# shaneson0/attacking_federate_learning

Measured on AMD Instinct MI355X. Metric: aggregation rounds/sec at N clients x D params (Bulyan), higher is better.
Workload: dtype f32 (Gram: fp16x2 split of every fp32 operand, 3 fp16 MFMAs per block, fp32/fp64 accumulate; <= 2e-7 of |gi||gj| vs f...

## Files before the change

### attacking_federate_learning_amd/csrc/gram_planes.hip

```cpp
#include "common.hpp"

#include <cstring>
#include <type_traits>

namespace byz {
namespace {

constexpr int kWgRows = 256;
constexpr int kWgCols = 128;
constexpr int kSlab = 128;
constexpr int kThreads = 512;
constexpr int kFragBytes = 1024;
constexpr int kRowBlocks = (kWgRows + kWgCols) / 32;
constexpr int kChunkCols = 8192;
constexpr int kChunkSteps = kChunkCols / 16;
constexpr int kFlushSteps = 16;
constexpr int kSpareRoundsPercent = 10;

typedef float f32x16 __attribute__((ext_vector_type(16)));
typedef float f32x4 __attribute__((ext_vector_type(4)));
typedef __bf16 bf16x8 __attribute__((ext_vector_type(8)));
typedef _Float16 f16x8 __attribute__((ext_vector_type(8)));
typedef uint32_t u32x4 __attribute__((ext_vector_type(4)));

__device__ __forceinline__ void split_bf16x3(const f32x4& lo4, const f32x4& hi4, u32x4& hp, u32x4& mp, u32x4& lp) {
    uint32_t xb[8], r1b[8], r2b[8];
#pragma unroll
    for (int e = 0; e < 8; ++e) {
        const float x = e < 4 ? lo4[e] : hi4[e - 4];
        xb[e] = __float_as_uint(x);
        const float r1 = x - __uint_as_float(xb[e] & 0xffff0000u);
        r1b[e] = __float_as_uint(r1);
        const float r2 = r1 - __uint_as_float(r1b[e] & 0xffff0000u);
        r2b[e] = __float_as_uint(r2);
    }
#pragma unroll
    for (int e = 0; e < 4; ++e) {
        hp[e] = __builtin_amdgcn_perm(xb[2 * e + 1], xb[2 * e], 0x07060302u);
        mp[e] = __builtin_amdgcn_perm(r1b[2 * e + 1], r1b[2 * e], 0x07060302u);
        lp[e] = __builtin_amdgcn_perm(r2b[2 * e + 1], r2b[2 * e], 0x07060302u);
    }
}

__device__ __forceinline__ void split_f16x2(const f32x4& lo4, const f32x4& hi4, float scale, u32x4& hp, u32x4& mp) {
    f16x8 h, m;
#pragma unroll
    for (int e = 0; e < 8; ++e) {
        const float x = (e < 4 ? lo4[e] : hi4[e - 4]) * scale;
        h[e] = static_cast<_Float16>(x);
        m[e] = static_cast<_Float16>(x - static_cast<float>(h[e]));
    }
    hp = __builtin_bit_cast(u32x4, h);
    mp = __builtin_bit_cast(u32x4, m);
}

__device__ __forceinline__ f32x4 load4_tail(const float* __restrict__ src, int64_t k, int64_t n_cols) {
    f32x4 v = {0.0f, 0.0f, 0.0f, 0.0f};
    if (k + 3 < n_cols) {
        v = *reinterpret_cast<const f32x4*>(src + k);
    } else {
        if (k + 0 < n_cols) v.x = src[k + 0];
        if (k + 1 < n_cols) v.y = src[k + 1];
        if (k + 2 < n_cols) v.z = src[k + 2];
    }
    return v;
}

constexpr int kSplitCols = 128;
__global__ __launch_bounds__(256) void plane_split_bf16_kernel(const float* __restrict__ G, int64_t n_rows, int64_t n_cols,
                                                               int64_t ld, const int32_t* __restrict__ row_index,
                                                               int64_t k0, int64_t n_steps, u32x4* __restrict__ planes) {
    __shared__ __attribute__((aligned(16))) float tile[32][kSplitCols + 4];
    const int tid = threadIdx.x;
    const int64_t rb = blockIdx.y;
    const int64_t step0 = static_cast<int64_t>(blockIdx.x) * (kSplitCols / 16);
    {
        const int r = tid >> 3, c = tid & 7;
        int64_t row = rb * 32 + r;
        if (row > n_rows - 1) row = n_rows - 1;
        if (row_index != nullptr) row = row_index[row];
        const float* src = G + row * ld;
#pragma unroll
        for (int p = 0; p < 4; ++p) {
            const int col = 4 * c + 32 * p;
            *reinterpret_cast<f32x4*>(&tile[r][col]) = load4_tail(src, k0 + step0 * 16 + col, n_cols);
        }
    }
    __syncthreads();
    const int lane = tid & 63, wave = tid >> 6;
#pragma unroll
    for (int i = 0; i < 2; ++i) {
        const int sl = 2 * wave + i;
        const int64_t step = step0 + sl;
        if (step >= n_steps) continue;
        const int row = lane & 31, kk = sl * 16 + 8 * (lane >> 5);
        const f32x4 lo4 = *reinterpret_cast<const f32x4*>(&tile[row][kk]);
        const f32x4 hi4 = *reinterpret_cast<const f32x4*>(&tile[row][kk + 4]);
        u32x4 h, m, l;
        split_bf16x3(lo4, hi4, h, m, l);
        u32x4* out = planes + ((rb * n_steps + step) * 3) * 64 + lane;
        out[0] = h;
        out[64] = m;
        out[128] = l;
    }
}

__global__ __launch_bounds__(256) void plane_split_f16_kernel(const float* __restrict__ G, int64_t n_rows, int64_t n_cols,
                                                              int64_t ld, const int32_t* __restrict__ row_index, int64_t k0,
                                                              int64_t n_steps, u32x4* __restrict__ planes,
                                                              double* __restrict__ unscale, int64_t rows_pad,
                                                              const int32_t* __restrict__ redo) {
    __shared__ __attribute__((aligned(16))) float tile[32][kSplitCols + 4];
    __shared__ float row_scale[32];
    const int tid = threadIdx.x;
    const int lane = tid & 63, wave = tid >> 6;
    const int listed = redo != nullptr ? redo[0] : 1;
    for (int item = redo != nullptr ? static_cast<int>(blockIdx.x) : 0; item < listed; item += static_cast<int>(gridDim.x)) {
    const int64_t rb = redo != nullptr ? redo[2 + 2 * item] : blockIdx.y;
    const int64_t chunk = redo != nullptr ? redo[1 + 2 * item] : blockIdx.x;
    const int r = tid >> 3, c = tid & 7;
    int64_t row = rb * 32 + r;
    if (row > n_rows - 1) row = n_rows - 1;
    if (row_index != nullptr) row = row_index[row];
    const float* src = G + row * ld;
    const int64_t kbeg = k0 + chunk * kChunkCols;
    {
        float mx = 0.0f;
        bool bad = false;
#pragma unroll 8
        for (int i = 0; i < kChunkCols / 32; ++i) {
            const f32x4 v = load4_tail(src, kbeg + 4 * c + 32 * i, n_cols);
#pragma unroll
            for (int e = 0; e < 4; ++e) {
                const float a = __builtin_fabsf(v[e]);
                bad = bad || !(a <= 3.0e38f);
                mx = __builtin_fmaxf(mx, a);
            }
        }
#pragma unroll
        for (int msk = 1; msk < 8; msk <<= 1) {
            mx = __builtin_fmaxf(mx, __shfl_xor(mx, msk, 64));
            bad = bad || (__shfl_xor(bad ? 1 : 0, msk, 64) != 0);
        }
        int shift = 0;
        if (!bad && mx > 0.0f) {
            shift = 14 - (static_cast<int>((__float_as_uint(mx) >> 23) & 0xffu) - 127);
            if (mx < 1.17549435e-38f) shift = 126;
            if (shift > 126) shift = 126;
            if (shift < -126) shift = -126;
        }
        if (c == 0) {
            row_scale[r] = __uint_as_float(static_cast<uint32_t>(shift + 127) << 23);
            unscale[chunk * rows_pad + rb * 32 + r] = __longlong_as_double(static_cast<long long>(1023 - shift) << 52);
        }
    }
    __syncthreads();
    const int64_t step_base = chunk * kChunkSteps;
    for (int sub = 0; sub < kChunkCols / kSplitCols; ++sub) {
        const int64_t step0 = step_base + sub * (kSplitCols / 16);
        if (step0 >= n_steps) break;
#pragma unroll
        for (int p = 0; p < 4; ++p) {
            const int col = 4 * c + 32 * p;
            *reinterpret_cast<f32x4*>(&tile[r][col]) = load4_tail(src, k0 + step0 * 16 + col, n_cols);
        }
        __syncthreads();
#pragma unroll
        for (int i = 0; i < 2; ++i) {
            const int sl = 2 * wave + i;
            const int64_t step = step0 + sl;
            if (step >= n_steps) continue;
            const int frow = lane & 31, kk = sl * 16 + 8 * (lane >> 5);
            const f32x4 lo4 = *reinterpret_cast<const f32x4*>(&tile[frow][kk]);
            const f32x4 hi4 = *reinterpret_cast<const f32x4*>(&tile[frow][kk + 4]);
            u32x4 h, m;
            split_f16x2(lo4, hi4, row_scale[frow], h, m);
            u32x4* out = planes + ((rb * n_steps + step) * 2) * 64 + lane;
            out[0] = h;
            out[64] = m;
        }
        __syncthreads();
    }
    if (redo == nullptr) break;
    __syncthreads();
    }
}

constexpr int kSampleGroups = 16;
__global__ __launch_bounds__(256) void plane_split_f16_stream_kernel(const float* __restrict__ G, int64_t n_rows, int64_t n_cols,
                                                                     int64_t ld, const int32_t* __restrict__ row_index, int64_t k0,
                                                                     int64_t n_steps, u32x4* __restrict__ planes,
                                                                     double* __restrict__ unscale, int64_t rows_pad,
                                                                     int32_t* __restrict__ redo) {
    __shared__ __attribute__((aligned(16))) float tile[2][32][kSplitCols + 4];
    __shared__ float row_scale[32];
    __shared__ int block_bad;
    const int tid = threadIdx.x;
    const int lane = tid & 63, wave = tid >> 6;
    const int64_t rb = blockIdx.y;
    const int64_t chunk = blockIdx.x;
    const int r = tid >> 3, c = tid & 7;
    int64_t row = rb * 32 + r;
    if (row > n_rows - 1) row = n_rows - 1;
    if (row_index != nullptr) row = row_index[row];
    const float* src = G + row * ld;
    const int64_t kbeg = k0 + chunk * kChunkCols;
    if (tid == 0) block_bad = 0;
    int shift = 0;
    {
        float mx = 0.0f;
#pragma unroll
        for (int g = 0; g < 2; ++g) {
            const int64_t k = kbeg + (2 * c + g) * (kChunkCols / kSampleGroups);
            const f32x4 a = load4_tail(src, k, n_cols), b = load4_tail(src, k + 4, n_cols);
#pragma unroll
            for (int e = 0; e < 4; ++e) mx = __builtin_fmaxf(mx, __builtin_fmaxf(__builtin_fabsf(a[e]), __builtin_fabsf(b[e])));
        }
#pragma unroll
        for (int msk = 1; msk < 8; msk <<= 1) mx = __builtin_fmaxf(mx, __shfl_xor(mx, msk, 64));
        if (mx >= 1.17549435e-38f && mx <= 3.0e38f) {
            shift = 9 - (static_cast<int>((__float_as_uint(mx) >> 23) & 0xffu) - 127);
            if (shift > 126) shift = 126;
            if (shift < -126) shift = -126;
        }
        if (c == 0) row_scale[r] = __uint_as_float(static_cast<uint32_t>(shift + 127) << 23);
    }
    const int64_t step_base = chunk * kChunkSteps;
    const float scale = __uint_as_float(static_cast<uint32_t>(shift + 127) << 23);
    float true_max = 0.0f;
    bool bad = false;
    f32x4 cur[4], nxt[4];
#pragma unroll
    for (int p = 0; p < 4; ++p) cur[p] = load4_tail(src, k0 + step_base * 16 + 4 * c + 32 * p, n_cols);
    __syncthreads();
    for (int sub = 0; sub < kChunkCols / kSplitCols; ++sub) {
        const int64_t step0 = step_base + sub * (kSplitCols / 16);
        if (step0 >= n_steps) break;
        const bool more = sub + 1 < kChunkCols / kSplitCols && step0 + kSplitCols / 16 < n_steps;
        if (more) {
#pragma unroll
            for (int p = 0; p < 4; ++p) nxt[p] = load4_tail(src, k0 + (step0 + kSplitCols / 16) * 16 + 4 * c + 32 * p, n_cols);
        }
        float (*t)[kSplitCols + 4] = tile[sub & 1];
#pragma unroll
        for (int p = 0; p < 4; ++p) {
            *reinterpret_cast<f32x4*>(&t[r][4 * c + 32 * p]) = cur[p];
#pragma unroll
            for (int e = 0; e < 4; ++e) {
                const float a = __builtin_fabsf(cur[p][e]);
                bad = bad || !(a <= 3.0e38f);
                true_max = __builtin_fmaxf(true_max, a);
            }
        }
        __syncthreads();
#pragma unroll
        for (int i = 0; i < 2; ++i) {
            const int sl = 2 * wave + i;
            const int64_t step = step0 + sl;
            if (step >= n_steps) continue;
            const int frow = lane & 31, kk = sl * 16 + 8 * (lane >> 5);
            const f32x4 lo4 = *reinterpret_cast<const f32x4*>(&t[frow][kk]);
            const f32x4 hi4 = *reinterpret_cast<const f32x4*>(&t[frow][kk + 4]);
            u32x4 h, m;
            split_f16x2(lo4, hi4, row_scale[frow], h, m);
            u32x4* out = planes + ((rb * n_steps + step) * 2) * 64 + lane;
            out[0] = h;
            out[64] = m;
        }
        if (more) {
#pragma unroll
            for (int p = 0; p < 4; ++p) cur[p] = nxt[p];
        }
    }
#pragma unroll
    for (int msk = 1; msk < 8; msk <<= 1) {
        true_max = __builtin_fmaxf(true_max, __shfl_xor(true_max, msk, 64));
        bad = bad || (__shfl_xor(bad ? 1 : 0, msk, 64) != 0);
    }
    const float scaled = true_max * scale;
    const bool holds = !bad && (true_max == 0.0f || (scaled >= 128.0f && scaled < 65536.0f));
    if (c == 0) {
        unscale[chunk * rows_pad + rb * 32 + r] = __longlong_as_double(static_cast<long long>(1023 - shift) << 52);
        if (!holds) block_bad = 1;
    }
    __syncthreads();
    if (tid == 0 && block_bad != 0) {
        const int at = atomicAdd(redo, 1);
        redo[1 + 2 * at] = static_cast<int32_t>(chunk);
        redo[2 + 2 * at] = static_cast<int32_t>(rb);
    }
}

template <int N>
__device__ __forceinline__ void wait_vmcnt() {
    asm volatile("s_waitcnt vmcnt(%0)" ::"n"(N) : "memory");
}
__device__ __forceinline__ void wait_vmcnt_dyn(int n) {
    switch (n) {
#define BYZ_W(k) case k: wait_vmcnt<k>(); break;
        BYZ_W(0) BYZ_W(3) BYZ_W(4) BYZ_W(5) BYZ_W(6) BYZ_W(8) BYZ_W(9) BYZ_W(10) BYZ_W(12) BYZ_W(15) BYZ_W(16) BYZ_W(18) BYZ_W(20) BYZ_W(24)
#undef BYZ_W
        default: wait_vmcnt<0>(); break;
    }
// ... 311 lines not shown

    const int tid = threadIdx.x;
    const int lane = tid & 63;
    const int wave = __builtin_amdgcn_readfirstlane(tid >> 6);
    const unsigned where = static_cast<unsigned>(__builtin_amdgcn_readfirstlane(my_unit->wave[wave].where));
    const int a_slot = static_cast<int>(where & 0xffu);
    const int b_slot = static_cast<int>((where >> 8) & 0xffu);
    unsigned live_blocks = (where >> 16) & 0xffu;
    const int row_in_slab = static_cast<int>((where >> 24) & 1u) * 64;
    const int col_in_slab = static_cast<int>((where >> 25) & 1u) * 64;
    const int sum_slot = __builtin_amdgcn_readfirstlane(my_unit->wave[wave].sum_slot);
    const bool live_wave = live_blocks != 0;

    const int step0 = chunk * kChunkSteps;
    int n_stages = static_cast<int>(n_steps) - step0;
    if (n_stages > kChunkSteps) n_stages = kChunkSteps;
    const int n_super = n_stages / 2;

    int64_t piece_off[kPerWave];
#pragma unroll
    for (int i = 0; i < kPerWave; ++i) {
        const int q = wave + NW * i;
        const int rbl = q / PLANES, piece = q % PLANES;
        const int64_t rb = __builtin_amdgcn_readfirstlane(my_unit->rb[rbl]);
        piece_off[i] = (((rb * n_steps + step0) * PLANES + piece) * 64) * 16;
    }
    const unsigned char* lane_base = reinterpret_cast<const unsigned char*>(planes) + lane * 16;
    auto dma_piece = [&](int s, int i) __attribute__((always_inline)) {
        unsigned char* dst = lds + (s % NBUF) * kStage + wave * kFragBytes;
        __builtin_amdgcn_global_load_lds(
            (const __attribute__((address_space(1))) void*)(lane_base + piece_off[i] + static_cast<int64_t>(s) * (PLANES * kFragBytes)),
            (__attribute__((address_space(3))) void*)(dst + i * NW * kFragBytes), 16, 0, 0);
    };
    auto dma = [&](int s) __attribute__((always_inline)) {
#pragma unroll
        for (int i = 0; i < kPerWave; ++i) dma_piece(s, i);
    };

    f32x4 acc[4][4], acc2[4][4];
#pragma unroll
    for (int m = 0; m < 4; ++m)
#pragma unroll
        for (int n = 0; n < 4; ++n)
#pragma unroll
            for (int e = 0; e < 4; ++e) {
                acc[m][n][e] = 0.0f;
                acc2[m][n][e] = 0.0f;
            }

    const int lane_in_image = (lane & 15) + 32 * ((lane >> 4) & 1);
    const int pair_half = lane >> 5;
    auto frag_at = [&](int sp, int rb32, int h, int p) __attribute__((always_inline)) -> frag_t {
        const unsigned char* at = lds + (2 * (sp % (NBUF / 2)) + pair_half) * kStage + rb32 * kRbBytes + p * kFragBytes +
                                  (lane_in_image + 16 * h) * 16;
        return *reinterpret_cast<const frag_t*>(at);
    };
    struct AFrags { frag_t v[2][4]; };
    struct BFrags { frag_t v[2][2]; };
    auto read_a = [&](int sp, AFrags& a, auto mask_c) __attribute__((always_inline)) {
        constexpr unsigned MASK = decltype(mask_c)::value;
#pragma unroll
        for (int p = 0; p < 2; ++p)
#pragma unroll
            for (int m = 0; m < 4; ++m)
                if (((MASK >> ((m / 2) * 2)) & 3u) != 0) a.v[p][m] = frag_at(sp, a_slot + m / 2, m % 2, p);
    };
    auto read_b = [&](int sp, int half, BFrags& b, auto mask_c) __attribute__((always_inline)) {
        constexpr unsigned MASK = decltype(mask_c)::value;
#pragma unroll
        for (int p = 0; p < 2; ++p)
#pragma unroll
            for (int n = 0; n < 2; ++n) b.v[p][n] = frag_at(sp, b_slot + half, n, p);
        (void)MASK;
    };
    auto multiply_half = [&](const AFrags& a, const BFrags& b, auto half_c, auto mask_c) __attribute__((always_inline)) {
        constexpr unsigned MASK = decltype(mask_c)::value;
        constexpr int HALF = decltype(half_c)::value;
        constexpr int pa[3] = {1, 0, 0};
        constexpr int pb[3] = {0, 1, 0};
#pragma unroll
        for (int t = 0; t < 3; ++t)
#pragma unroll
            for (int m = 0; m < 4; ++m)
#pragma unroll
                for (int n = 0; n < 2; ++n)
                    if (((MASK >> ((m / 2) * 2 + HALF)) & 1u) != 0)
                        acc[m][2 * HALF + n] = __builtin_amdgcn_mfma_f32_16x16x32_f16(a.v[pa[t]][m], b.v[pb[t]][n], acc[m][2 * HALF + n], 0, 0, 0);
    };
    auto flush = [&](int sp) __attribute__((always_inline)) {
        if ((sp + 1) % kSuperFlush == 0) {
#pragma unroll
            for (int m = 0; m < 4; ++m)
#pragma unroll
                for (int n = 0; n < 4; ++n)
#pragma unroll
                    for (int e = 0; e < 4; ++e) {
                        acc2[m][n][e] += acc[m][n][e];
                        acc[m][n][e] = 0.0f;
                    }
        }
    };

    for (int a = 0; a < NBUF && a < n_stages; ++a) dma(a);
    {
        const int issued = n_stages < NBUF ? n_stages : NBUF;
        wait_vmcnt_dyn((issued > 2 ? issued - 2 : 0) * kPerWave);
    }
    asm volatile("s_barrier" ::: "memory");
    auto k_loop = [&](auto mask_c) __attribute__((always_inline)) {
        constexpr unsigned MASK = decltype(mask_c)::value;
        constexpr bool kLive = MASK != 0;
        constexpr std::integral_constant<int, 0> h0{};
        constexpr std::integral_constant<int, 1> h1{};
        AFrags a0, a1;
        BFrags b0, b1;
        if (kLive && n_super > 0) {
            read_a(0, a0, mask_c);
            if ((MASK & 5u) != 0) read_b(0, 0, b0, mask_c);
        }
        auto super = [&](int sp, AFrags& a, AFrags& an) __attribute__((always_inline)) {
            if (kLive) {
                if ((MASK & 10u) != 0) read_b(sp, 1, b1, mask_c);
                if ((MASK & 5u) != 0) multiply_half(a, b0, h0, mask_c);
            }
            {
                const int last = 2 * sp + 5 < n_stages - 1 ? 2 * sp + 5 : n_stages - 1;
                const int ahead = last - (2 * sp + 3);
                if (2 * sp + 7 < n_stages) wait_vmcnt<2 * kPerWave>();
                else wait_vmcnt_dyn((ahead > 0 ? ahead : 0) * kPerWave);
            }
            asm volatile("s_waitcnt lgkmcnt(0)\n\ts_barrier" ::: "memory");
            if (2 * sp + NBUF < n_stages) dma(2 * sp + NBUF);
            if (2 * sp + NBUF + 1 < n_stages) dma(2 * sp + NBUF + 1);
            if (kLive) {
                if (sp + 1 < n_super) {
                    read_a(sp + 1, an, mask_c);
                    if ((MASK & 5u) != 0) read_b(sp + 1, 0, b0, mask_c);
                }
                if ((MASK & 10u) != 0) multiply_half(a, b1, h1, mask_c);
                flush(sp);
            }
        };
        auto super8 = [&](int sp, AFrags& a, AFrags& an, auto pos_c) __attribute__((always_inline)) {
            constexpr int POS = decltype(pos_c)::value;
            constexpr bool FRESH = POS == 0, FLUSHING = POS == 7;
            constexpr int pa[3] = {1, 0, 0};
            constexpr int pb[3] = {0, 1, 0};
            const f32x4 zero4 = {0.0f, 0.0f, 0.0f, 0.0f};
            auto walk_n = [](int k) __attribute__((always_inline)) { return ((k / 2) & 1) ? 1 - k % 2 : k % 2; };
#pragma unroll
            for (int k = 0; k < 8; ++k) {
                const int m = k / 2, n = walk_n(k);
                if (k % 2 == 0) b1.v[k / 4][m % 2] = frag_at(sp, b_slot + 1, m % 2, k / 4);
#pragma unroll
                for (int t = 0; t < 3; ++t) {
                    acc[m][n] = __builtin_amdgcn_mfma_f32_16x16x32_f16(a.v[pa[t]][m], b0.v[pb[t]][n], (FRESH && t == 0) ? zero4 : acc[m][n], 0, 0, 0);
                    __builtin_amdgcn_sched_barrier(0);
                }
            }
            wait_vmcnt<2 * kPerWave>();
            asm volatile("s_waitcnt lgkmcnt(0)\n\ts_barrier" ::: "memory");
#pragma unroll
            for (int k = 0; k < 8; ++k) {
                const int m = k / 2, n = walk_n(k);
                if (k < 6) {
                    dma_piece(2 * sp + NBUF + k / 3, k % 3);
#pragma unroll
                    for (int r = 2 * k; r < 2 * k + 2; ++r) {
                        if (r < 8) an.v[r / 4][r % 4] = frag_at(sp + 1, a_slot + (r % 4) / 2, (r % 4) % 2, r / 4);
                        else b0.v[(r - 8) / 2][(r - 8) % 2] = frag_at(sp + 1, b_slot, (r - 8) % 2, (r - 8) / 2);
                    }
                }
#pragma unroll
                for (int t = 0; t < 3; ++t) {
                    acc[m][2 + n] = __builtin_amdgcn_mfma_f32_16x16x32_f16(a.v[pa[t]][m], b1.v[pb[t]][n], (FRESH && t == 0) ? zero4 : acc[m][2 + n], 0, 0, 0);
                    __builtin_amdgcn_sched_barrier(0);
                }
                if constexpr (FLUSHING) {
#pragma unroll
                    for (int e = 0; e < 4; ++e) acc2[m][k % 2][e] += acc[m][k % 2][e];
                }
            }
            if constexpr (FLUSHING) {
#pragma unroll
                for (int m = 0; m < 4; ++m)
#pragma unroll
                    for (int n = 2; n < 4; ++n)
#pragma unroll
                        for (int e = 0; e < 4; ++e) acc2[m][n][e] += acc[m][n][e];
            }
        };
        int sp = 0;
        if constexpr (MASK == 15u) {
            bool any = false;
            for (; 2 * (sp + 7) + NBUF + 1 < n_stages && sp + 8 < n_super; sp += 8) {
                super8(sp + 0, a0, a1, std::integral_constant<int, 0>{});
                super8(sp + 1, a1, a0, std::integral_constant<int, 1>{});
                super8(sp + 2, a0, a1, std::integral_constant<int, 2>{});
                super8(sp + 3, a1, a0, std::integral_constant<int, 3>{});
                super8(sp + 4, a0, a1, std::integral_constant<int, 4>{});
                super8(sp + 5, a1, a0, std::integral_constant<int, 5>{});
                super8(sp + 6, a0, a1, std::integral_constant<int, 6>{});
                super8(sp + 7, a1, a0, std::integral_constant<int, 7>{});
                any = true;
            }
            if (any) {
#pragma unroll
                for (int m = 0; m < 4; ++m)
#pragma unroll
                    for (int n = 0; n < 4; ++n)
#pragma unroll
                        for (int e = 0; e < 4; ++e) acc[m][n][e] = 0.0f;
            }
        }
        for (; sp + 1 < n_super; sp += 2) {
            super(sp, a0, a1);
            super(sp + 1, a1, a0);
        }
        if (sp < n_super) super(sp, a0, a1);
    };
    switch (live_blocks) {
        case 0u: k_loop(std::integral_constant<unsigned, 0u>{}); break;
        case 1u: k_loop(std::integral_constant<unsigned, 1u>{}); break;
        case 3u: k_loop(std::integral_constant<unsigned, 3u>{}); break;
        case 13u: k_loop(std::integral_constant<unsigned, 13u>{}); break;
        default: live_blocks = 15u; k_loop(std::integral_constant<unsigned, 15u>{}); break;
    }
    auto block_live = [&](int m, int n) __attribute__((always_inline)) { return ((live_blocks >> ((m / 2) * 2 + n / 2)) & 1u) != 0; };

    if constexpr (DEFER) {
        if (live_wave) {
            const bool unflushed = (n_super % kSuperFlush) != 0;
            float* out = chunk_sums + (static_cast<int64_t>(chunk) * n_sum_slots + sum_slot) * (kSlab * kSlab);
            float* rag = ragged_sums + static_cast<int64_t>(sum_slot) * (kSlab * kSlab);
#pragma unroll
            for (int m = 0; m < 4; ++m)
#pragma unroll
                for (int n = 0; n < 4; ++n) {
                    if (!block_live(m, n)) continue;
                    const int j = col_in_slab + 16 * n + (lane & 15);
#pragma unroll
                    for (int e = 0; e < 4; ++e) {
                        const int i = row_in_slab + 16 * m + 4 * (lane >> 4) + e;
                        out[i * kSlab + j] = acc2[m][n][e];
                        if (unflushed) rag[i * kSlab + j] = acc[m][n][e];
                    }
                }
        }
        __syncthreads();
        if (tid == 0) __hip_atomic_fetch_add(done, 1, __ATOMIC_RELAXED, __HIP_MEMORY_SCOPE_AGENT);
        return;
    }
    bool lost = false;
    if (chunk > 0) {
        if (tid == 0) {
            unsigned spins = 0;
            while (__hip_atomic_load(tickets + t_list, __ATOMIC_RELAXED, __HIP_MEMORY_SCOPE_AGENT) != chunk) {
                __builtin_amdgcn_s_sleep(8);
                if (++spins > (1u << 26)) {
                    lost = true;
                    break;
                }
            }
            __builtin_amdgcn_fence(__ATOMIC_ACQUIRE, "agent");
        }
        lost = __syncthreads_or(lost ? 1 : 0) != 0;
    }
    if (lost) {
        if (tid == 0) atomicOr(device_status, kStatusLostTicket);
    } else if (live_wave) {
        const bool slab_live = chunk > 0 || slab_live0 != 0;
        const int slab = __builtin_amdgcn_readfirstlane(my_unit->wave[wave].slab);
        const int ti = slab & 0xffff, tj = slab >> 16;
        double* out = partial + (static_cast<int64_t>(ti) * (ti + 1) / 2 + tj) * (kSlab * kSlab);
        const double* un = unscale + static_cast<int64_t>(chunk) * rows_pad;
#pragma unroll
        for (int m = 0; m < 4; ++m)
#pragma unroll
            for (int n = 0; n < 4; ++n) {
                if (!block_live(m, n)) continue;
                const int j = col_in_slab + 16 * n + (lane & 15);
                const double uj = un[static_cast<int64_t>(tj) * kSlab + j];
#pragma unroll
                for (int e = 0; e < 4; ++e) {
                    const int i = row_in_slab + 16 * m + 4 * (lane >> 4) + e;
                    double v = static_cast<double>(acc2[m][n][e]);
                    v += static_cast<double>(acc[m][n][e]);
                    v *= un[static_cast<int64_t>(ti) * kSlab + i] * uj;
                    if (slab_live) v += out[i * kSlab + j];
                    out[i * kSlab + j] = v;
                }
            }
    }
    asm volatile("s_waitcnt vmcnt(0)" ::: "memory");
    __syncthreads();
    if (tid == 0) {
        __builtin_amdgcn_fence(__ATOMIC_RELEASE, "agent");
        asm volatile("s_waitcnt vmcnt(0)" ::: "memory");
        __hip_atomic_store(tickets + t_list, chunk + 1, __ATOMIC_RELAXED, __HIP_MEMORY_SCOPE_AGENT);
        __hip_atomic_fetch_add(done, 1, __ATOMIC_RELAXED, __HIP_MEMORY_SCOPE_AGENT);
    }
}

constexpr int kReduceRun = 8;
__global__ __launch_bounds__(256) void chunk_reduce_kernel(const float* __restrict__ chunk_sums, const float* __restrict__ ragged_sums,
                                                           int n_sum_slots, int n_chunks, int ragged_chunk,
                                                           const int2* __restrict__ slot_slab, const double* __restrict__ unscale,
                                                           int64_t rows_pad, double* __restrict__ partial, int slab_live0,
                                                           int n_blocks32) {
    typedef double f64x4 __attribute__((ext_vector_type(4)));
    const int slot = blockIdx.x;
    const int2 tt = slot_slab[slot];
    const int ti = tt.x, tj = tt.y;
    if (ti < 0) return;
    double* out = partial + (static_cast<int64_t>(ti) * (ti + 1) / 2 + tj) * (kSlab * kSlab);
    const int64_t slab_stride = static_cast<int64_t>(n_sum_slots) * (kSlab * kSlab);
    const float* in = chunk_sums + static_cast<int64_t>(slot) * (kSlab * kSlab);
    const float* rag = ragged_sums + static_cast<int64_t>(slot) * (kSlab * kSlab);
    const int i = static_cast<int>(blockIdx.y) * 32 + (threadIdx.x >> 3), j = (threadIdx.x & 7) * 4;
    for (int jb = 0; jb < kSlab; jb += 32) {
        const int jj = jb + j;
        if (n_blocks32 >= 0) {
            const int rblk = ti * 4 + (i >> 5), cblk = tj * 4 + (jj >> 5);
            if (!(rblk < n_blocks32 && cblk <= rblk)) continue;
        }
        const int idx = i * kSlab + jj;
        f64x4 v = {0.0, 0.0, 0.0, 0.0};
        bool live = slab_live0 != 0;
        if (live) v = *reinterpret_cast<const f64x4*>(out + idx);
        for (int c0 = 0; c0 < n_chunks; c0 += kReduceRun) {
            f32x4 p[kReduceRun];
            double ui[kReduceRun];
            f64x4 uj[kReduceRun];
#pragma unroll
            for (int k = 0; k < kReduceRun; ++k) {
                const int c = c0 + k < n_chunks ? c0 + k : n_chunks - 1;
                p[k] = *reinterpret_cast<const f32x4*>(in + c * slab_stride + idx);
                const double* un = unscale + static_cast<int64_t>(c) * rows_pad;
                ui[k] = un[static_cast<int64_t>(ti) * kSlab + i];
                uj[k] = *reinterpret_cast<const f64x4*>(un + static_cast<int64_t>(tj) * kSlab + jj);
            }
#pragma unroll
            for (int k = 0; k < kReduceRun; ++k) {
                if (c0 + k >= n_chunks) break;
                f64x4 q = {static_cast<double>(p[k][0]), static_cast<double>(p[k][1]), static_cast<double>(p[k][2]),
                           static_cast<double>(p[k][3])};
                if (c0 + k == ragged_chunk) {
                    const f32x4 r = *reinterpret_cast<const f32x4*>(rag + idx);
                    q[0] += static_cast<double>(r[0]); q[1] += static_cast<double>(r[1]);
                    q[2] += static_cast<double>(r[2]); q[3] += static_cast<double>(r[3]);
                }
#pragma unroll
                for (int e = 0; e < 4; ++e) {
                    q[e] *= ui[k] * uj[k][e];
                    v[e] = live ? q[e] + v[e] : q[e];
                }
                live = true;
            }
        }
        *reinterpret_cast<f64x4*>(out + idx) = v;
    }
}

}

bool gram_planes_enabled() { return env_int("BYZ_GRAM_PLANES", 1) != 0; }

void build_gram_units(int64_t t128, int64_t n_blocks32, bool diagonal_units, int share_count, int share_index,
                      std::vector<GramUnit>& units, std::vector<int32_t>& slot_slab) {
    units.clear();
    slot_slab.clear();
    const int64_t t256 = ceil_div(t128, 2);
    auto live_mask = [&](int64_t ti, int64_t tj, int row64, int col64) -> uint32_t {
        if (!(tj <= ti && ti < t128)) return 0u;
        if (n_blocks32 < 0) return 15u;
        uint32_t mask = 0;
        for (int m = 0; m < 2; ++m)
            for (int n = 0; n < 2; ++n) {
                const int64_t rblk = ti * 4 + row64 * 2 + m, cblk = tj * 4 + col64 * 2 + n;
                if (rblk < n_blocks32 && cblk <= rblk) mask |= 1u << (m * 2 + n);
            }
        return mask;
    };
    auto set_wave = [&](GramUnit& u, int wave, int a_slot, int b_slot, int64_t ti, int64_t tj, int row64, int col64,
                        int64_t sum_slot) {
        const uint32_t mask = live_mask(ti, tj, row64, col64);
        GramUnitWave& w = u.wave[wave];
        w.where = static_cast<uint32_t>(a_slot) | static_cast<uint32_t>(b_slot) << 8 | mask << 16 |
                  static_cast<uint32_t>(row64) << 24 | static_cast<uint32_t>(col64) << 25;
        w.sum_slot = mask != 0 ? static_cast<int32_t>(sum_slot) : 0;
        w.slab = mask != 0 ? static_cast<int32_t>(ti | tj << 16) : 0;
    };
    auto slab_slot = [](int64_t ti, int64_t tj) { return ti * (ti + 1) / 2 + tj; };
    int64_t position = 0;
    auto plain = [&](int64_t bi, int64_t tj, bool d1) {
        if (position++ % share_count != share_index) return;
        const int64_t t_list = static_cast<int64_t>(units.size());
        GramUnit u{};
        for (int s = 0; s < 12; ++s) u.rb[s] = static_cast<int32_t>(s < 8 ? bi * 8 + s : tj * 4 + (s - 8));
        for (int wave = 0; wave < 8; ++wave) {
            const int wr = wave / 2, wc = wave % 2;
            const int64_t ti = 2 * bi + wr / 2;
            set_wave(u, wave, 2 * wr, 8 + 2 * wc, ti, tj, wr % 2, wc, diagonal_units ? slab_slot(ti, tj) : 2 * t_list + wr / 2);
        }
        if (d1) set_wave(u, 1, 4, 4, 2 * bi + 1, 2 * bi + 1, 0, 0, slab_slot(2 * bi + 1, 2 * bi + 1));
        units.push_back(u);
        if (!diagonal_units)
            for (int sel = 0; sel < 2; ++sel) {
                const int64_t ti = 2 * bi + sel;
                const bool live = tj <= ti && ti < t128;
                slot_slab.push_back(static_cast<int32_t>(live ? ti : -1));
                slot_slab.push_back(static_cast<int32_t>(live ? tj : -1));
            }
    };
    auto d2 = [&](int64_t first, int64_t count) {
        static const int partial_wave[3] = {3, 7, 5};
        GramUnit u{};
        for (int s = 0; s < 12; ++s) u.rb[s] = static_cast<int32_t>(first * 8 + 4);
        for (int64_t k = 0; k < count; ++k) {
            const int64_t bi = first + k, t = 2 * bi + 1;
            for (int s = 0; s < 4; ++s) u.rb[4 * k + s] = static_cast<int32_t>(bi * 8 + 4 + s);
            set_wave(u, static_cast<int>(k), static_cast<int>(4 * k + 2), static_cast<int>(4 * k), t, t, 1, 0, slab_slot(t, t));
            set_wave(u, partial_wave[k], static_cast<int>(4 * k + 2), static_cast<int>(4 * k + 2), t, t, 1, 1, slab_slot(t, t));
        }
        units.push_back(u);
    };
    const int64_t full_blocks = t128 / 2;
    for (int64_t b0 = 0; b0 < t256; b0 += 4)
        for (int64_t tj = 0; tj < t128 && tj <= 2 * (b0 + 3) + 1; ++tj)
            for (int64_t bi = b0; bi < b0 + 4 && bi < t256; ++bi) {
                if (tj > 2 * bi + 1) continue;
                if (!diagonal_units) {
                    plain(bi, tj, false);
                } else if (tj == 2 * bi + 1) {
                    if (bi % 3 == 2 || bi == full_blocks - 1) d2(bi - bi % 3, bi % 3 + 1);
                } else {
                    plain(bi, tj, tj == 2 * bi);
                }
            }
    if (diagonal_units)
        for (int64_t ti = 0; ti < t128; ++ti)
            for (int64_t tj = 0; tj <= ti; ++tj) {
                slot_slab.push_back(static_cast<int32_t>(ti));
                slot_slab.push_back(static_cast<int32_t>(tj));
            }
}

int launch_gram_planes(byz_ctx* ctx, const float* G, int64_t n_rows, int64_t n_cols, int64_t ld, const int32_t* row_index,
                       double* slabs, int share_count, int share_index, uint8_t* owned_host, bool f16, hipStream_t stream) {
    const int64_t t128 = ceil_div(n_rows, kSlab);
    const int64_t t256 = ceil_div(t128, 2);
    const int64_t rows_pad = t256 * kWgRows;
    bool defer = f16 && env_int("BYZ_GRAM_DEFER", 1) != 0;
    const int n_blocks32 = env_int("BYZ_GRAM_BLOCK_SKIP", 1) != 0 ? static_cast<int>(ceil_div(n_rows, 32)) : -1;
    auto ensure_list = [&](bool diagonal_units) -> int {
        const int64_t order_key = static_cast<int64_t>((f16 ? 1 : 0) + (diagonal_units ? 2 : 0)) * (1ll << 40) + share_count * 65536 + share_index;
        const int64_t blocks_key = f16 ? n_blocks32 : -2;
        if (ctx->plane_order_T != t128 || ctx->plane_order_share != order_key || ctx->plane_order_blocks != blocks_key) {
            ctx->plane_order_host.clear();
            if (f16) {
                if (t128 > 0x7fff) {
                    set_error("gram: more than 32767 slabs per side");
                    return BYZ_E_UNSUPPORTED;
                }
                std::vector<GramUnit> units;
                std::vector<int32_t> slot_slab;
                build_gram_units(t128, n_blocks32, diagonal_units, share_count, share_index, units, slot_slab);
                ctx->plane_units = static_cast<int64_t>(units.size());
                ctx->plane_sum_slots = static_cast<int64_t>(slot_slab.size() / 2);
                ctx->plane_order_host.resize(units.size() * kGramUnitWords);
                if (!units.empty()) std::memcpy(ctx->plane_order_host.data(), units.data(), units.size() * sizeof(GramUnit));
                ctx->plane_order_host.insert(ctx->plane_order_host.end(), slot_slab.begin(), slot_slab.end());
            } else {
                int64_t position = 0;
                auto push = [&](int64_t bi, int64_t tj) {
                    if (position++ % share_count != share_index) return;
                    ctx->plane_order_host.push_back(static_cast<int32_t>(bi));
                    ctx->plane_order_host.push_back(static_cast<int32_t>(tj));
                };
                const int64_t S = ceil_div(t128, 8);
                for (int64_t I = 0; I < S; ++I)
                    for (int64_t J = 0; J <= I; ++J)
                        for (int64_t bi = I * 4; bi < I * 4 + 4 && bi < t256; ++bi)
                            for (int64_t tj = J * 8; tj < J * 8 + 8 && tj <= 2 * bi + 1 && tj < t128; ++tj) push(bi, tj);
                ctx->plane_units = static_cast<int64_t>(ctx->plane_order_host.size() / 2);
                ctx->plane_sum_slots = 0;
            }
            BYZ_TRY(ctx->plane_order.ensure(ctx->plane_order_host.size() * sizeof(int32_t) + 16));
            BYZ_HIP(hipMemcpyAsync(ctx->plane_order.ptr, ctx->plane_order_host.data(),
                                   ctx->plane_order_host.size() * sizeof(int32_t), hipMemcpyHostToDevice, stream));
            BYZ_HIP(hipStreamSynchronize(stream));
            ctx->plane_order_T = t128;
            ctx->plane_order_share = order_key;
            ctx->plane_order_blocks = blocks_key;
        }
        return BYZ_OK;
    };
    const bool diagonal_units = defer && share_count == 1 && n_blocks32 >= 0;
    BYZ_TRY(ensure_list(diagonal_units));
    int64_t n_tiles = ctx->plane_units;
    int64_t n_sum_slots = ctx->plane_sum_slots;
    const int32_t* slot_slab_host = ctx->plane_order_host.data() + n_tiles * kGramUnitWords;
    if (owned_host != nullptr) {
        if (f16) {
            for (int64_t s = 0; s < n_sum_slots; ++s) {
                const int64_t ti = slot_slab_host[2 * s], tj = slot_slab_host[2 * s + 1];
                if (ti >= 0) owned_host[ti * (ti + 1) / 2 + tj] = 1;
            }
        } else {
            for (int64_t t = 0; t < n_tiles; ++t) {
                const int64_t bi = ctx->plane_order_host[2 * t], tj = ctx->plane_order_host[2 * t + 1];
                for (int64_t ti = 2 * bi; ti < 2 * bi + 2 && ti < t128; ++ti)
                    if (tj <= ti) owned_host[ti * (ti + 1) / 2 + tj] = 1;
            }
        }
    }
    if (n_tiles == 0) return BYZ_OK;

    const int n_planes = f16 ? 2 : 3;
    size_t free_b = 0, total_b = 0;
    BYZ_HIP(hipMemGetInfo(&free_b, &total_b));
    int64_t budget = static_cast<int64_t>(env_int("BYZ_GRAM_PLANE_MB", 16384)) << 20;
    const int64_t have = static_cast<int64_t>(ctx->gram_planes.bytes);
    if (budget > have + static_cast<int64_t>(free_b / 2)) budget = have + static_cast<int64_t>(free_b / 2);
    int64_t chunks_per_sc = budget / (rows_pad * 2 * n_planes * kChunkCols);
    const int64_t chunks_total = ceil_div(n_cols, kChunkCols);
    if (chunks_per_sc > chunks_total) chunks_per_sc = chunks_total;
    if (chunks_per_sc < 1) {
        set_error("gram: no room for one 8192-column chunk of 16-bit planes (%lld rows)", (long long)rows_pad);
        return BYZ_E_HIP;
    }
    const int64_t n_sc = ceil_div(chunks_total, chunks_per_sc);
    chunks_per_sc = ceil_div(chunks_total, n_sc);
    const int64_t sc_cols = chunks_per_sc * kChunkCols;
    BYZ_TRY(ctx->gram_planes.ensure(static_cast<size_t>(rows_pad) * 2 * n_planes * sc_cols));
    double* unscale = nullptr;
    if (f16) {
        BYZ_TRY(ctx->plane_unscale.ensure(static_cast<size_t>(rows_pad) * chunks_per_sc * sizeof(double)));
        unscale = ctx->plane_unscale.as<double>();
    }
    u32x4* planes = ctx->gram_planes.as<u32x4>();
    float* chunk_sums = nullptr;
    float* ragged_sums = nullptr;
    if (defer) {
        const size_t per_chunk = static_cast<size_t>(n_sum_slots) * kSlab * kSlab * sizeof(float);
        const size_t want = per_chunk * static_cast<size_t>(chunks_per_sc + 1);
        size_t free_now = 0, total_now = 0;
        BYZ_HIP(hipMemGetInfo(&free_now, &total_now));
        if (want > ctx->gram_chunk_sums.bytes && want - ctx->gram_chunk_sums.bytes > free_now / 2) defer = false;
        if (!defer && diagonal_units) {
            BYZ_TRY(ensure_list(false));
            n_tiles = ctx->plane_units;
            n_sum_slots = ctx->plane_sum_slots;
        }
    }
    if (defer) {
        const size_t per_chunk = static_cast<size_t>(n_sum_slots) * kSlab * kSlab * sizeof(float);
        BYZ_TRY(ctx->gram_chunk_sums.ensure(per_chunk * static_cast<size_t>(chunks_per_sc + 1)));
        chunk_sums = ctx->gram_chunk_sums.as<float>();
        ragged_sums = chunk_sums + (per_chunk / sizeof(float)) * static_cast<size_t>(chunks_per_sc);
    }
    auto kernel16 = defer ? &gram_planes16_kernel<6, true> : &gram_planes16_kernel<6, false>;
    const void* kernel = f16 ? reinterpret_cast<const void*>(kernel16) : reinterpret_cast<const void*>(&gram_planes_kernel<4>);
    const size_t lds_bytes = static_cast<size_t>(f16 ? 6 : 4) * kRowBlocks * n_planes * kFragBytes;
    BYZ_HIP(allow_dynamic_lds(ctx, kernel, static_cast<int>(lds_bytes)));
    const int round_size = env_int("BYZ_GRAM_ROUND", ctx->num_cus / 8);
    const int run = round_size > 0 ? round_size : ctx->num_cus / 8;
    const int64_t per_xcd = ceil_div(n_tiles, 8);
    for (int64_t sc = 0; sc < n_sc; ++sc) {
        const int64_t k0 = sc * sc_cols;
        const int64_t cols = n_cols - k0 < sc_cols ? n_cols - k0 : sc_cols;
        const int64_t n_steps = ceil_div(cols, 32) * 2;
        const int64_t n_chunks = ceil_div(n_steps, kChunkSteps);
        {
            KernelTimer t(ctx, BYZ_K_PLANE_SPLIT, stream);
            if (f16) {
                const dim3 grid(static_cast<unsigned>(n_chunks), static_cast<unsigned>(rows_pad / 32));
                if (env_int("BYZ_GRAM_SPLIT_TWO_PASS", 0) != 0) {
                    plane_split_f16_kernel<<<grid, 256, 0, stream>>>(G, n_rows, n_cols, ld, row_index, k0, n_steps, planes,
                                                                     unscale, rows_pad, nullptr);
                } else {
                    const int64_t pairs = n_chunks * (rows_pad / 32);
                    BYZ_TRY(ctx->split_redo.ensure(static_cast<size_t>(1 + 2 * pairs) * sizeof(int32_t)));
                    int32_t* redo = ctx->split_redo.as<int32_t>();
                    BYZ_HIP(hipMemsetAsync(redo, 0, sizeof(int32_t), stream));
                    plane_split_f16_stream_kernel<<<grid, 256, 0, stream>>>(G, n_rows, n_cols, ld, row_index, k0, n_steps, planes,
                                                                            unscale, rows_pad, redo);
                    BYZ_TRY(check_launch("plane_split_f16_stream_kernel"));
                    const int64_t fix = pairs < 4096 ? pairs : 4096;
                    plane_split_f16_kernel<<<static_cast<unsigned>(fix), 256, 0, stream>>>(G, n_rows, n_cols, ld, row_index, k0,
                                                                                           n_steps, planes, unscale, rows_pad, redo);
                }
            } else {
                const dim3 grid(static_cast<unsigned>(ceil_div(n_steps, kSplitCols / 16)), static_cast<unsigned>(rows_pad / 32));
                plane_split_bf16_kernel<<<grid, 256, 0, stream>>>(G, n_rows, n_cols, ld, row_index, k0, n_steps, planes);
            }
            BYZ_TRY(check_launch("plane_split_kernel"));
        }
        {
            int64_t rounds_per_xcd = 0;
            if (f16) {
                rounds_per_xcd = ceil_div(ceil_div(n_tiles * n_chunks, run), 8);
                rounds_per_xcd += rounds_per_xcd * kSpareRoundsPercent / 100;
            }
            const int64_t grid = f16 ? 8 * run * rounds_per_xcd : 8 * per_xcd * n_chunks;
            const size_t ticket_ints = static_cast<size_t>(n_tiles + 9 + 8 * rounds_per_xcd);
            BYZ_TRY(ctx->gram_tickets.ensure(ticket_ints * sizeof(int)));
            int* tickets = ctx->gram_tickets.as<int>();
            BYZ_HIP(hipMemsetAsync(tickets, 0, ticket_ints * sizeof(int), stream));
            KernelTimer t(ctx, BYZ_K_GRAM, stream);
            if (grid > 0x7fffffff) {
                set_error("gram: grid too large");
                return BYZ_E_UNSUPPORTED;
            }
            const int slab_live0 = sc > 0 ? 1 : 0;
            if (!f16) {
                gram_planes_kernel<4><<<static_cast<unsigned>(grid), kThreads, lds_bytes, stream>>>(
                    planes, n_steps, slabs, static_cast<int>(n_tiles), ctx->plane_order.as<int2>(), static_cast<int>(n_chunks), tickets,
                    round_size, static_cast<int>(t128), slab_live0, n_blocks32, device_status_word(ctx));
            } else {
                kernel16<<<static_cast<unsigned>(grid), kThreads, lds_bytes, stream>>>(
                    planes, n_steps, unscale, rows_pad, slabs, static_cast<int>(n_tiles), ctx->plane_order.as<GramUnit>(),
                    static_cast<int>(n_chunks), tickets, round_size, run, slab_live0, static_cast<int>(n_sum_slots),
                    device_status_word(ctx), chunk_sums, ragged_sums);
            }
            BYZ_TRY(check_launch("gram_planes_kernel"));
        }
        if (defer) {
            KernelTimer t(ctx, BYZ_K_GRAM_REDUCE, stream);
            const int ragged_chunk = (n_steps % kChunkSteps) % kFlushSteps != 0 ? static_cast<int>(n_chunks) - 1 : -1;
            const int2* slot_slab = reinterpret_cast<const int2*>(ctx->plane_order.as<GramUnit>() + n_tiles);
            chunk_reduce_kernel<<<dim3(static_cast<unsigned>(n_sum_slots), 4), 256, 0, stream>>>(
                chunk_sums, ragged_sums, static_cast<int>(n_sum_slots), static_cast<int>(n_chunks), ragged_chunk, slot_slab,
                unscale, rows_pad, slabs, sc > 0 ? 1 : 0, n_blocks32);
            BYZ_TRY(check_launch("chunk_reduce_kernel"));
        }
    }
    return BYZ_OK;
}

}
```

Measured before the change: 2.096.

## Restructure chunk reduce to stage unscale exponents in LDS and loop all column blocks

The chunk reduction kernel now handles all four 32-column blocks per thread inside one loop. It stages the per-chunk unscale factors as int16 exponents in shared memory in batches of 128 chunks, and rebuilds each scale as a power of two by bit construction instead of loading fp64 ui/uj from global memory on every chunk. Workgroups whose quarter has no live blocks exit early. The change assumes unscale values are exact powers of two, and adds shared-memory staging with barriers plus more registers for four accumulators; the live-mask helper is also moved to a shared header.

```diff
diff --git a/attacking_federate_learning_amd/csrc/chunk_sums_map.hpp b/attacking_federate_learning_amd/csrc/chunk_sums_map.hpp
--- /dev/null
+++ b/attacking_federate_learning_amd/csrc/chunk_sums_map.hpp
@@ -0,0 +1,52 @@
+#pragma once
+
+#include <cstdint>
+
+#if defined(__HIPCC__)
+#define BYZ_SUMS_FN __host__ __device__ __forceinline__
+#else
+#define BYZ_SUMS_FN inline
+#endif
+
+namespace byz {
+namespace chunk_sums {
+
+constexpr int kSlabEdge = 128;
+constexpr int kSlotFloats = kSlabEdge * kSlabEdge;
+
+struct Element {
+    int i, j;
+};
+
+BYZ_SUMS_FN Element element_of(int row_in_slab, int col_in_slab, int m, int n, int lane, int e) {
+    Element at;
+    at.i = row_in_slab + 16 * m + 4 * (lane >> 4) + e;
+    at.j = col_in_slab + 16 * n + (lane & 15);
+    return at;
+}
+
+BYZ_SUMS_FN int offset_of(Element at) { return at.i * kSlabEdge + at.j; }
+
+BYZ_SUMS_FN Element reduce_entry(int quarter, int tid, int n) {
+    Element at;
+    at.i = 32 * quarter + (tid >> 3);
+    at.j = 32 * n + 4 * (tid & 7);
+    return at;
+}
+
+BYZ_SUMS_FN bool mask_has(unsigned live_blocks, int m, int n) { return ((live_blocks >> ((m / 2) * 2 + n / 2)) & 1u) != 0; }
+
+BYZ_SUMS_FN bool block_computed(int64_t rblk, int64_t cblk, int64_t n_blocks32) {
+    return n_blocks32 < 0 || (rblk < n_blocks32 && cblk <= rblk);
+}
+
+BYZ_SUMS_FN unsigned quadrant_mask(int64_t ti, int64_t tj, int row64, int col64, int64_t n_blocks32) {
+    unsigned mask = 0;
+    for (int m = 0; m < 2; ++m)
+        for (int n = 0; n < 2; ++n)
+            if (block_computed(ti * 4 + row64 * 2 + m, tj * 4 + col64 * 2 + n, n_blocks32)) mask |= 1u << (m * 2 + n);
+    return mask;
+}
+
+}
+}
diff --git a/attacking_federate_learning_amd/csrc/gram_planes.hip b/attacking_federate_learning_amd/csrc/gram_planes.hip
--- a/attacking_federate_learning_amd/csrc/gram_planes.hip
+++ b/attacking_federate_learning_amd/csrc/gram_planes.hip
@@ -1,4 +1,5 @@
 #include "common.hpp"
+#include "chunk_sums_map.hpp"
 
 #include <cstring>
 #include <type_traits>
@@ -916,64 +917,91 @@
     }
 }
 
-constexpr int kReduceRun = 8;
+constexpr int kReduceRun = 4;
+constexpr int kReduceBatch = 128;
 __global__ __launch_bounds__(256) void chunk_reduce_kernel(const float* __restrict__ chunk_sums, const float* __restrict__ ragged_sums,
                                                            int n_sum_slots, int n_chunks, int ragged_chunk,
                                                            const int2* __restrict__ slot_slab, const double* __restrict__ unscale,
                                                            int64_t rows_pad, double* __restrict__ partial, int slab_live0,
                                                            int n_blocks32) {
     typedef double f64x4 __attribute__((ext_vector_type(4)));
+    typedef int16_t i16x4 __attribute__((ext_vector_type(4)));
+    __shared__ __attribute__((aligned(16))) int16_t exponent[kReduceBatch][32 + kSlab];
     const int slot = blockIdx.x;
     const int2 tt = slot_slab[slot];
     const int ti = tt.x, tj = tt.y;
     if (ti < 0) return;
+    const int tid = threadIdx.x, quarter = blockIdx.y;
+    bool live_n[4], any = false;
+#pragma unroll
+    for (int n = 0; n < 4; ++n) {
+        live_n[n] = chunk_sums::block_computed(ti * 4 + quarter, tj * 4 + n, n_blocks32);
+        any = any || live_n[n];
+    }
+    if (!any) return;
     double* out = partial + (static_cast<int64_t>(ti) * (ti + 1) / 2 + tj) * (kSlab * kSlab);
-    const int64_t slab_stride = static_cast<int64_t>(n_sum_slots) * (kSlab * kSlab);
-    const float* in = chunk_sums + static_cast<int64_t>(slot) * (kSlab * kSlab);
-    const float* rag = ragged_sums + static_cast<int64_t>(slot) * (kSlab * kSlab);
-    const int i = static_cast<int>(blockIdx.y) * 32 + (threadIdx.x >> 3), j = (threadIdx.x & 7) * 4;
-    for (int jb = 0; jb < kSlab; jb += 32) {
-        const int jj = jb + j;
-        if (n_blocks32 >= 0) {
-            const int rblk = ti * 4 + (i >> 5), cblk = tj * 4 + (jj >> 5);
-            if (!(rblk < n_blocks32 && cblk <= rblk)) continue;
-        }
-        const int idx = i * kSlab + jj;
-        f64x4 v = {0.0, 0.0, 0.0, 0.0};
-        bool live = slab_live0 != 0;
-        if (live) v = *reinterpret_cast<const f64x4*>(out + idx);
-        for (int c0 = 0; c0 < n_chunks; c0 += kReduceRun) {
-            f32x4 p[kReduceRun];
-            double ui[kReduceRun];
-            f64x4 uj[kReduceRun];
+    const int64_t slab_stride = static_cast<int64_t>(n_sum_slots) * chunk_sums::kSlotFloats;
+    const float* in = chunk_sums + static_cast<int64_t>(slot) * chunk_sums::kSlotFloats;
+    const float* rag = ragged_sums + static_cast<int64_t>(slot) * chunk_sums::kSlotFloats;
+    int idx[4];
+#pragma unroll
+    for (int n = 0; n < 4; ++n) idx[n] = chunk_sums::offset_of(chunk_sums::reduce_entry(quarter, tid, n));
+    const int row_in_quarter = tid >> 3, col_in_block = 4 * (tid & 7);
+
+    f64x4 v[4];
+    bool live = slab_live0 != 0;
+#pragma unroll
+    for (int n = 0; n < 4; ++n) {
+        v[n] = f64x4{0.0, 0.0, 0.0, 0.0};
+        if (live && live_n[n]) v[n] = *reinterpret_cast<const f64x4*>(out + idx[n]);
+    }
+    for (int b0 = 0; b0 < n_chunks; b0 += kReduceBatch) {
+        const int nb = n_chunks - b0 < kReduceBatch ? n_chunks - b0 : kReduceBatch;
+        if (b0 > 0) __syncthreads();
+        for (int t = tid; t < nb * (32 + kSlab); t += 256) {
+            const int c = t / (32 + kSlab), k = t % (32 + kSlab);
+            const int64_t row = k < 32 ? static_cast<int64_t>(ti) * kSlab + 32 * quarter + k : static_cast<int64_t>(tj) * kSlab + (k - 32);
+            const int32_t w = reinterpret_cast<const int32_t*>(unscale)[2 * (static_cast<int64_t>(b0 + c) * rows_pad + row) + 1];
+            exponent[c][k] = static_cast<int16_t>(((w >> 20) & 0x7ff) - 1023);
+        }
+        __syncthreads();
+        for (int c0 = 0; c0 < nb; c0 += kReduceRun) {
+            f32x4 p[kReduceRun][4];
 #pragma unroll
             for (int k = 0; k < kReduceRun; ++k) {
-                const int c = c0 + k < n_chunks ? c0 + k : n_chunks - 1;
-                p[k] = *reinterpret_cast<const f32x4*>(in + c * slab_stride + idx);
-                const double* un = unscale + static_cast<int64_t>(c) * rows_pad;
-                ui[k] = un[static_cast<int64_t>(ti) * kSlab + i];
-                uj[k] = *reinterpret_cast<const f64x4*>(un + static_cast<int64_t>(tj) * kSlab + jj);
+                const int c = b0 + (c0 + k < nb ? c0 + k : nb - 1);
+#pragma unroll
+                for (int n = 0; n < 4; ++n)
+                    if (live_n[n]) p[k][n] = *reinterpret_cast<const f32x4*>(in + c * slab_stride + idx[n]);
             }
 #pragma unroll
             for (int k = 0; k < kReduceRun; ++k) {
-                if (c0 + k >= n_chunks) break;
-                f64x4 q = {static_cast<double>(p[k][0]), static_cast<double>(p[k][1]), static_cast<double>(p[k][2]),
-                           static_cast<double>(p[k][3])};
-                if (c0 + k == ragged_chunk) {
-                    const f32x4 r = *reinterpret_cast<const f32x4*>(rag + idx);
-                    q[0] += static_cast<double>(r[0]); q[1] += static_cast<double>(r[1]);
-                    q[2] += static_cast<double>(r[2]); q[3] += static_cast<double>(r[3]);
-                }
-#pragma unroll
-                for (int e = 0; e < 4; ++e) {
-                    q[e] *= ui[k] * uj[k][e];
-                    v[e] = live ? q[e] + v[e] : q[e];
+                if (c0 + k >= nb) break;
+                const int ei = exponent[c0 + k][row_in_quarter];
+#pragma unroll
+                for (int n = 0; n < 4; ++n) {
+                    if (!live_n[n]) continue;
+                    const i16x4 ej = *reinterpret_cast<const i16x4*>(&exponent[c0 + k][32 + 32 * n + col_in_block]);
+                    double q[4] = {static_cast<double>(p[k][n][0]), static_cast<double>(p[k][n][1]),
+                                   static_cast<double>(p[k][n][2]), static_cast<double>(p[k][n][3])};
+                    if (b0 + c0 + k == ragged_chunk) {
+                        const f32x4 r = *reinterpret_cast<const f32x4*>(rag + idx[n]);
+#pragma unroll
+                        for (int e = 0; e < 4; ++e) q[e] += static_cast<double>(r[e]);
+                    }
+#pragma unroll
+                    for (int e = 0; e < 4; ++e) {
+                        q[e] *= __longlong_as_double(static_cast<long long>(ei + static_cast<int>(ej[e]) + 1023) << 52);
+                        v[n][e] = live ? q[e] + v[n][e] : q[e];
+                    }
                 }
                 live = true;
             }
         }
-        *reinterpret_cast<f64x4*>(out + idx) = v;
-    }
+    }
+#pragma unroll
+    for (int n = 0; n < 4; ++n)
+        if (live_n[n]) *reinterpret_cast<f64x4*>(out + idx[n]) = v[n];
 }
 
 }
@@ -987,14 +1015,7 @@
     const int64_t t256 = ceil_div(t128, 2);
     auto live_mask = [&](int64_t ti, int64_t tj, int row64, int col64) -> uint32_t {
         if (!(tj <= ti && ti < t128)) return 0u;
-        if (n_blocks32 < 0) return 15u;
-        uint32_t mask = 0;
-        for (int m = 0; m < 2; ++m)
-            for (int n = 0; n < 2; ++n) {
-                const int64_t rblk = ti * 4 + row64 * 2 + m, cblk = tj * 4 + col64 * 2 + n;
-                if (rblk < n_blocks32 && cblk <= rblk) mask |= 1u << (m * 2 + n);
-            }
-        return mask;
+        return chunk_sums::quadrant_mask(ti, tj, row64, col64, n_blocks32);
     };
     auto set_wave = [&](GramUnit& u, int wave, int a_slot, int b_slot, int64_t ti, int64_t tj, int row64, int col64,
                         int64_t sum_slot) {
```

After: 2.105 (median of 6 runs). About the same (+0.4%).
